# KrishnaswamyLab/MELD

Hardware: AMD Instinct MI355X
Metric: cells/sec through MELD.fit_transform (kNN+Chebyshev) (higher is better)
Workload: dtype f64

## Files before the change

### include/meld_hip.h

```cpp
#ifndef MELD_HIP_H
#define MELD_HIP_H

#include <stddef.h>
#include <stdint.h>

#ifdef __cplusplus
extern "C" {
#endif

#define MELD_OK 0
#define MELD_ERR_INVALID (-1)
#define MELD_ERR_UNSUPPORTED (-2)
#define MELD_ERR_HIP (-3)

typedef void* meld_stream_t;

int meld_abi_version(void);
const char* meld_last_error(void);
int meld_device_count(void);


int meld_knn_padded_dim(int d);
int meld_knn_tile_refs(void);
int meld_knn_block_queries(void);
int meld_knn_row_capacity(int ksel);
double meld_knn_error_coef(int d);

int meld_col_sums_f64(const double* X, int64_t N, int d, double* sums, meld_stream_t stream);
size_t meld_col_stats_temp_bytes(int d);
int meld_col_stats_f64(const double* X, int64_t N, int d, double* sums, double* mins, double* maxs, void* temp, size_t temp_bytes,
                       meld_stream_t stream);

int meld_knn_prepare_refs(const double* X, int64_t N, int d, const double* mean, int KP, float* Rt,
                          float* norm2, float* norm2_max, meld_stream_t stream);
int meld_knn_prepare_queries(const double* X, int64_t N, int d, const double* mean, int KP,
                             int64_t q_begin, int64_t q_count, float* Q, meld_stream_t stream);

int meld_knn_topk(const float* Q, const float* Rt, int64_t n_ref, int KP, int64_t q_count, int ksel,
                  int32_t* cand_idx, float* cand_d2, int32_t* cand_cnt, meld_stream_t stream);

int meld_knn16_kblocks(int d);
int meld_knn16_tile_refs(void);
int meld_knn16_split_dims(int d);
int meld_frame_max_dims(void);
int meld_cov_sample_f64(const double* X, int64_t N, int d, const double* mean, int64_t stride, double* cov, meld_stream_t stream);
int meld_rotate_rows_f64(const double* X, int64_t N, int d, const double* mean, const double* At, double* out, meld_stream_t stream);
int meld_knn16_block_queries(void);
int meld_knn16_row_capacity(int ksel);
double meld_knn16_error_coef(int nprod, int d);
double meld_knn16_error_coef_const(int nprod, int d);
double meld_knn16_error_coef_lin(int nprod);
size_t meld_knn16_tile_bytes(int d);
size_t meld_knn16_query_bytes(int d);
int meld_knn16_prepare(const double* X, int64_t N, int d, const double* mean, int64_t q_begin,
                       int64_t q_count, void* Rt16, void* Q16, float* Qn, float* norm2, float* norm2_max,
                       float* scale_info, meld_stream_t stream);
int meld_knn16_prepare_scaled(const double* X, int64_t N, int d, const double* mean, const double* col_min, const double* col_max,
                              int64_t q_begin, int64_t q_count, void* Rt16, void* Q16, float* Qn, float* norm2, float* norm2_max,
                              float* scale_info, meld_stream_t stream);
int meld_knn16_prepare_fused(const double* X, int64_t N, int d, const double* mean, const double* col_min, const double* col_max,
                             void* Rt16, void* Q16, float* Qn, float* norm2, float* norm2_max, float* scale_info, void* temp,
                             meld_stream_t stream);
size_t meld_knn16_bounds_bytes(int64_t n_ref, int64_t q_count);
size_t meld_knn16_bounds_temp_bytes(int64_t n_ref, int d, int64_t q_count);
int meld_knn16_bounds(const double* X, int64_t N, int d, const double* mean, const float* scale_info,
                      const float* norm2_max, const void* Rt16, int64_t q_begin, int64_t q_count,
                      const float* thr_seed, const float* q_norm2 ,
                      int nprod, void* temp, void* lb2, meld_stream_t stream);
int meld_knn16_tile_spheres(const double* X, int64_t N, int d, const double* mean, const float* scale_info, void* temp,
                            int64_t tile_begin, int64_t tile_count, meld_stream_t stream);
int meld_knn16_sphere_layout(int64_t n_ref, int d, int64_t* rows, int64_t* row_bytes);
int meld_knn16_bounds_from_spheres(const double* X, int64_t N, int d, const double* mean, const float* scale_info,
                      const float* norm2_max, const void* Rt16, int64_t q_begin, int64_t q_count,
                      const float* thr_seed, const float* q_norm2 ,
                      int nprod, void* temp, void* lb2, meld_stream_t stream);
int meld_knn16_prepare_cross(const double* X, int64_t n_refs, int64_t n_total, int d, const double* mean, int64_t q_begin,
                             int64_t q_count, void* Rt16, void* Q16, float* Qn, float* norm2, float* norm2_max,
                             float* scale_info, meld_stream_t stream);
int meld_knn16_prepare_rows(const double* X, int64_t N, int d, const double* mean, const float* scale_info,
                            int64_t q_begin, const int32_t* rows, int64_t n_rows, void* Q16, float* Qn,
                            meld_stream_t stream);
int meld_knn16_research_thresholds(const int32_t* rows, int64_t n_rows, int64_t q_begin, const int32_t* cand_cnt,
                                   const float* cand_d2, int cap, int ksel, const float* norm2, const float* norm2_max,
                                   double err_coef, double err_lin, double err3, const float* scale_info, float* thr,
                                   meld_stream_t stream);
int meld_knn16_seed_thresholds_mfma(const void* Q16, const float* Qn, const void* Rt16, const float* scale_info,
                                    const float* norm2_max, int64_t n_ref, int d, int64_t q_begin, int64_t q_count,
                                    int knn, double radius_factor, int nprod, int side_tiles, float* thr_init,
                                    meld_stream_t stream);
int meld_knn16_topk(const void* Q16, const float* Qn, const void* Rt16, const float* scale_info,
                    int64_t n_ref, int d, int64_t q_count, int ksel, int nprod, int n_slices, const void* lb2,
                    const float* norm2_max, int64_t q_begin, const float* thr_init, int knn, double radius_factor,
                    int32_t* cand_idx, float* cand_d2, int32_t* cand_cnt, float* cand_thr,
                    uint64_t* tiles_done ,
                    const int32_t* block_order ,
                    meld_stream_t stream);
int meld_knn16_block_work(const void* lb2, const float* thr_seed, int64_t n_ref, int d, int64_t q_count, int nprod,
                          const float* norm2_max, const float* scale_info, int32_t* work, meld_stream_t stream);
int meld_knn16_step_lists(const void* lb2, const float* thr_seed, int64_t n_ref, int d, int64_t q_count, int nprod,
// ... 340 lines not shown
```

### meld_amd/_lib.py

```python
from __future__ import annotations

from ._options import is_set, opt

import ctypes as C
import os

_HERE = os.path.dirname(os.path.abspath(__file__))
LIB_NAME = "libmeld_hip.so"
LIB_PATH = os.path.join(_HERE, LIB_NAME)

_i32, _i64, _f64, _sz, _ptr = C.c_int, C.c_int64, C.c_double, C.c_size_t, C.c_void_p

SIGNATURES = {
    "meld_abi_version": (_i32, []),
    "meld_last_error": (C.c_char_p, []),
    "meld_device_count": (_i32, []),
    "meld_knn_padded_dim": (_i32, [_i32]),
    "meld_knn_tile_refs": (_i32, []),
    "meld_knn_block_queries": (_i32, []),
    "meld_knn_row_capacity": (_i32, [_i32]),
    "meld_col_sums_f64": (_i32, [_ptr, _i64, _i32, _ptr, _ptr]),
    "meld_col_stats_temp_bytes": (_sz, [_i32]),
    "meld_col_stats_f64": (_i32, [_ptr, _i64, _i32, _ptr, _ptr, _ptr, _ptr, _sz, _ptr]),
    "meld_knn_prepare_refs": (_i32, [_ptr, _i64, _i32, _ptr, _i32, _ptr, _ptr, _ptr, _ptr]),
# ... 85 lines not shown
    "meld_csr_transpose_keys": (_i32, [_ptr, _ptr, _ptr, _i32, _i64, _ptr, _ptr, _ptr]),
    "meld_csr_rows_to_dense_f64": (_i32, [_ptr, _ptr, _ptr, _i32, _i64, _i64, _i64, _ptr, _i64, _ptr]),
    "meld_csr_bucket_slots": (_i32, []),
    "meld_coo_scatter_rows": (_i32, [_ptr, _ptr, _i64, _i64, _i64, _ptr, _ptr, _ptr, _ptr]),
    "meld_coo_emit_scatter": (_i32, [_i64, _ptr, _ptr, _i32, _i32, _ptr, _ptr, _i32, _ptr, _ptr, _ptr, _i64, _ptr, _ptr, _ptr, _ptr]),
    "meld_coo_emit_scatter_listed": (_i32, [_ptr, _i32, _ptr, _ptr, _i32, _i32, _ptr, _ptr, _i32, _ptr, _ptr, _ptr, _i64, _ptr, _ptr, _ptr, _ptr]),
    "meld_coo_partition_remote": (_i32, [_ptr, _ptr, _i64, _i64, _i32, _i32, _i64, _ptr, _ptr, _ptr]),
    "meld_csr_rows_sort_merge": (_i32, [_ptr, _i64, _ptr, _ptr, _ptr, _ptr, _i32, _f64, _ptr]),
    "meld_csr_compact_rows": (_i32, [_ptr, _i64, _ptr, _ptr, _ptr, _ptr, _ptr]),
    "meld_csr_rows_sort_merge_sums": (_i32, [_ptr, _i64, _ptr, _ptr, _ptr, _ptr, _i32, _f64, _f64, _ptr, _ptr]),
    "meld_csr_compact_rows_anisotropy": (_i32, [_ptr, _i64, _ptr, _ptr, _ptr, _ptr, _ptr, _f64, _ptr, _ptr]),
    "meld_csr_compact_rows_sums": (_i32, [_ptr, _i64, _ptr, _ptr, _ptr, _ptr, _f64, _ptr, _ptr]),
    "meld_csr_row_sums": (_i32, [_ptr, _ptr, _i64, _f64, _ptr, _ptr]),
    "meld_csr_anisotropy": (_i32, [_ptr, _ptr, _ptr, _i64, _ptr, _i64, _f64, _ptr]),
    "meld_csr_anisotropy_degrees": (_i32, [_ptr, _ptr, _ptr, _i64, _ptr, _i64, _f64, _ptr, _ptr]),
    "meld_extend_rows_temp_bytes": (_sz, [_i64, _i64]),
    "meld_extend_rows": (_i32, [_ptr, _ptr, _i64, _i64, _i64, _i64, _ptr, _ptr, _ptr, _ptr, _ptr, _sz, _ptr]),
    "meld_extend_apply": (_i32, [_ptr, _ptr, _ptr, _ptr, _i64, _ptr, _i64, _i32, _ptr, _ptr, _ptr]),
    "meld_spmm_dot_slots": (_i32, []),
    "meld_cheby_step": (_i32, [_ptr, _i32, _ptr, _i64, _ptr, _ptr, _ptr, _f64, _f64, _f64, _f64, _ptr, _ptr]),
    "meld_lanczos_steps": (_i32, [_ptr, _ptr, _ptr, _ptr, _ptr, _ptr, _ptr, _i32, _i32, _ptr, _ptr, _ptr]),
    "meld_lanczos_spmv": (_i32, [_ptr, _ptr, _i64, _ptr, _ptr, _ptr, _ptr, _ptr]),
    "meld_lanczos_alpha": (_i32, [_ptr, _ptr, _ptr, _ptr, _i32, _ptr]),
    "meld_lanczos_axpy": (_i32, [_ptr, _ptr, _i64, _ptr, _ptr, _ptr]),
    "meld_lanczos_beta": (_i32, [_ptr, _ptr, _ptr, _ptr, _i32, _ptr]),
    "meld_lanczos_fold": (_i32, [_ptr, _ptr, _ptr, _ptr, _i32, _ptr]),
    "meld_lanczos_axpy3": (_i32, [_ptr, _ptr, _ptr, _i64, _ptr, _ptr, _ptr]),
    "meld_pt_geometry": (_i32, [_ptr, _ptr, _ptr, _ptr]),
    "meld_pt_num_blocks": (_i32, [_i64]),
    "meld_pt_seg_len": (_i64, [_i32]),
    "meld_pt_stream_len": (_i64, [_i64, _i32]),
    "meld_pt_desc_len": (_i64, [_i32]),
    "meld_pt_build": (_i32, [_ptr, _ptr, _ptr, _i64, _i64, _i64, _i32, _ptr, _ptr, _ptr, _ptr]),
    "meld_cheby_step_wide": (_i32, [_ptr, _i32, _ptr, _i64, _ptr, _ptr, _f64, _f64, _f64, _ptr]),
    "meld_block_max_blocks": (_i32, []),
    "meld_block_gram_f64": (_i32, [_ptr, _i64, _ptr, _i64, _i64, _i32, _ptr, _i32, _ptr, _ptr]),
    "meld_block_rotate_f64": (_i32, [_ptr, _i64, _ptr, _i64, _i32, _ptr, _i64, _ptr]),
    "meld_block_residuals_f64": (_i32, [_ptr, _ptr, _i64, _ptr, _i64, _i32, _ptr, _i32, _ptr, _ptr]),
    "meld_kmeans_max_blocks": (_i32, []),
    "meld_kmeans_assign": (_i32, [_ptr, _i64, _i32, _ptr, _i32, _ptr, _ptr, _ptr, _ptr, _i32, _ptr]),
    "meld_kmeans_wide_max_d": (_i32, []),
    "meld_kmeans_wide_max_k": (_i32, []),
    "meld_kmeans_wide_assign": (_i32, [_ptr, _i64, _i64, _i32, _ptr, _i32, _ptr, _ptr, _ptr, _ptr]),
    "meld_kmeans_wide_sums": (_i32, [_ptr, _i64, _i64, _i32, _ptr, _ptr, _i32, _ptr, _ptr]),
    "meld_scale_f64": (_i32, [_ptr, _f64, _ptr, _i64, _ptr]),
    "meld_axpby_f64": (_i32, [_f64, _ptr, _f64, _ptr, _i64, _ptr, _ptr]),
    "meld_normalize_rows_l1": (_i32, [_ptr, _ptr, _i64, _i32, _ptr]),
    "meld_assign_nearest": (_i32, [_ptr, _i64, _i32, _ptr, _i32, _ptr, _ptr, _ptr, _ptr]),
    "meld_chain_order": (_i32, [_ptr, _i64, _i32, _i32, _ptr, _ptr]),
    "meld_gather_rows_f64": (_i32, [_ptr, _ptr, _i64, _i32, _ptr, _ptr]),
    "meld_frame_max_dims": (_i32, []),
    "meld_cov_sample_f64": (_i32, [_ptr, _i64, _i32, _ptr, _i64, _ptr, _ptr]),
    "meld_rotate_rows_f64": (_i32, [_ptr, _i64, _i32, _ptr, _ptr, _ptr, _ptr]),
    "meld_argsort_u32_temp_bytes": (_sz, [_i64]),
    "meld_argsort_u32": (_i32, [_ptr, _i64, _i32, _ptr, _ptr, _ptr, _sz, _ptr]),
    "meld_order_starts": (_i32, [_ptr, _i64, _i32, _ptr, _ptr]),
    "meld_order_pick_centroids": (_i32, [_ptr, _i64, _i32, _ptr, _ptr, _i32, _i32, _ptr, _ptr]),
    "meld_order_update_keys": (_i32, [_ptr, _ptr, _ptr, _i64, _i32, _ptr]),
    "meld_rccl_available": (_i32, []),
    "meld_rccl_unique_id": (_i32, [_ptr]),
    "meld_rccl_comm_create": (_i32, [_ptr, _i32, _i32, _ptr]),
    "meld_rccl_comm_destroy": (_i32, [_ptr]),
    "meld_rccl_all_gather": (_i32, [_ptr, _ptr, _ptr, _sz, _ptr]),
    "meld_rccl_all_reduce_sum_f64": (_i32, [_ptr, _ptr, _sz, _ptr]),
    "meld_cheby_run": (_i32, [_ptr, _ptr, _i64, _i64, _i32, _ptr, _ptr, _ptr, _ptr, _i32, _f64, _f64, _ptr, _ptr]),
    "meld_lanczos_steps_sharded": (_i32, [_ptr, _ptr, _i64, _i64, _ptr, _ptr, _ptr, _ptr, _ptr, _ptr, _ptr, _i32, _i32, _ptr]),
    "meld_factorize_max_groups": (_i32, []),
    "meld_factorize_max_words": (_i32, []),
    "meld_factorize_temp_bytes": (_sz, [_i64]),
    "meld_factorize_labels": (_i32, [_ptr, _i64, _i32, _ptr, _sz, _ptr, _ptr]),
    "meld_factorize_codes": (_i32, [_ptr, _i64, _ptr, _ptr, _ptr]),
    "meld_indicator_signal": (_i32, [_ptr, _ptr, _ptr, _i64, _i64, _i32, _ptr, _ptr]),
    "meld_scatter_rows_f64": (_i32, [_ptr, _ptr, _i64, _i32, _ptr, _ptr]),
    "meld_cc_round": (_i32, [_ptr, _ptr, _i64, _ptr, _ptr, _ptr]),
    "meld_cc_minima": (_i32, [_ptr, _ptr, _i64, _ptr, _ptr, _ptr, _ptr]),
    "meld_cc_labels": (_i32, [_ptr, _ptr, _ptr, _ptr, _ptr, _i64, _ptr, _ptr, _ptr]),
    "meld_subgraph_count": (_i32, [_ptr, _ptr, _ptr, _i64, _ptr, _ptr]),
    "meld_subgraph_fill": (_i32, [_ptr, _ptr, _ptr, _ptr, _i64, _ptr, _ptr, _ptr, _ptr]),
    "meld_diffuse_max_cols": (_i32, []),
    "meld_diffuse_step": (_i32, [_ptr, _ptr, _ptr, _ptr, _ptr, _i64, _ptr, _i64, _ptr, _i64, _i32, _ptr]),
    "meld_minplus_max_cols": (_i32, []),
    "meld_minplus_step": (_i32, [_ptr, _ptr, _ptr, _i64, _ptr, _i64, _ptr, _i64, _i32, _ptr, _ptr]),
    "meld_edge_lengths_l2": (_i32, [_ptr, _ptr, _i64, _ptr, _i64, _i32, _ptr, _ptr]),
    "meld_landmark_max": (_i32, []),
    "meld_landmark_merge_count": (_i32, [_ptr, _ptr, _i64, _i64, _ptr, _i32, _ptr, _i32, _ptr, _ptr, _ptr]),
    "meld_landmark_merge_fill": (_i32, [_ptr, _ptr, _ptr, _i64, _ptr, _ptr, _ptr, _ptr, _ptr, _ptr]),
    "meld_landmark_gram": (_i32, [_ptr, _ptr, _ptr, _i64, _ptr, _ptr, _ptr, _i32, _ptr, _ptr, _ptr, _ptr]),
    "meld_smacof_max_dim": (_i32, []),
    "meld_smacof_step": (_i32, [_ptr, _i64, _i32, _i32, _ptr, _ptr, _ptr, _ptr]),
    "meld_louvain_lanes": (_i32, [_i64, _i64]),
    "meld_louvain_move_blocks": (_i64, [_i64, _i32]),
    "meld_louvain_move": (_i32, [_ptr, _ptr, _ptr, _i64, _ptr, _ptr, _ptr, _ptr, _f64, _f64, _i32, _i32, _ptr, _ptr, _ptr, _ptr, _ptr, _ptr, _ptr]),
    "meld_louvain_totals": (_i32, [_ptr, _ptr, _i64, _i64, _ptr, _ptr, _ptr, _ptr]),
    "meld_louvain_heads": (_i32, [_ptr, _ptr, _i64, _ptr, _ptr]),
    "meld_louvain_renumber": (_i32, [_ptr, _ptr, _ptr, _ptr, _i64, _ptr, _ptr, _ptr]),
    "meld_louvain_contract_keys": (_i32, [_ptr, _ptr, _i64, _ptr, _ptr, _ptr]),
    "meld_modularity_terms": (_i32, [_ptr, _ptr, _ptr, _i64, _ptr, _ptr, _ptr, _ptr]),
}


class PtLayout(C.Structure):

    _fields_ = [("blk_row", _ptr), ("blk_ntile", _ptr), ("blk_ndist", _ptr), ("seg", _ptr), ("list_cols", _ptr),
                ("pval", _ptr), ("pidx", _ptr), ("nb", C.c_int32), ("pval32", _ptr), ("stream_len", C.c_int64), ("cdesc", _ptr)]


# ... 42 lines not shown
```

### meld_amd/csrc/frame.hip

```cpp
#include "common.hpp"

namespace meld {

constexpr int FR_ROWS = 64;
constexpr int FR_DMAX = 64;

__global__ __launch_bounds__(256) void cov_sample_kernel(const double* __restrict__ X, int64_t n_s, int64_t stride, int d,
                                                         const double* __restrict__ mean, double* __restrict__ out) {
  __shared__ double sx[FR_ROWS][FR_DMAX + 1];
  const int tid = threadIdx.x;
  const int64_t s0 = (int64_t)blockIdx.x * FR_ROWS;
  const int cnt = (int)min((int64_t)FR_ROWS, n_s - s0);
  for (int u = tid; u < FR_ROWS * d; u += 256) {
    const int r = u / d, k = u - r * d;
    sx[r][k] = r < cnt ? X[(s0 + r) * stride * d + k] - mean[k] : 0.0;
  }
  __syncthreads();
  for (int p = tid; p < d * d; p += 256) {
    const int i = p / d, j = p - i * d;
    if (j < i) continue;
    double acc = 0.0;
    for (int r = 0; r < FR_ROWS; ++r) acc = fma(sx[r][i], sx[r][j], acc);
    atomicAdd(out + p, acc);
  }
}

typedef double f64x8 __attribute__((ext_vector_type(8)));
typedef const __attribute__((address_space(4))) f64x8* const_f64x8_ptr;
constexpr int FR_LD = FR_DMAX + 1;
constexpr int FR_NQ = FR_ROWS * FR_DMAX / 256;
constexpr int FR_CPG = FR_DMAX / 4;
__global__ __launch_bounds__(256) void rotate_rows_kernel(const double* __restrict__ X, int64_t N, int d, const double* __restrict__ mean,
                                                          const double* __restrict__ At, double* __restrict__ out, int64_t tiles_per_wg) {
  __shared__ double sx[FR_ROWS][FR_LD];
  const int tid = threadIdx.x, lane = tid & 63;
  const int w = __builtin_amdgcn_readfirstlane(tid >> 6);
  const int cpg = (d + 3) >> 2;
  const int j0 = w * cpg;
  const int k8n = (d + 7) >> 3;
  const double mk = (lane < d) ? mean[lane] : 0.0;
  const int64_t n_tiles = (N + FR_ROWS - 1) / FR_ROWS;
  const int64_t t_begin = (int64_t)blockIdx.x * tiles_per_wg, t_end = min(n_tiles, t_begin + tiles_per_wg);
  double xv[FR_NQ];
  auto fetch = [&](int64_t t) __attribute__((always_inline)) {
    const int64_t row0 = t * FR_ROWS;
#pragma unroll
    for (int q = 0; q < FR_NQ; ++q) {
      const int u = tid + 256 * q, rr = u >> 6, k = u & 63;
      xv[q] = (t < t_end && row0 + rr < N && k < d) ? X[(row0 + rr) * d + k] : mk;
    }
  };
  fetch(t_begin);
  for (int64_t t = t_begin; t < t_end; ++t) {
    const int64_t row0 = t * FR_ROWS;
    const int cnt = (int)min((int64_t)FR_ROWS, N - row0);
    __syncthreads();
#pragma unroll
    for (int q = 0; q < FR_NQ; ++q) {
      const int u = tid + 256 * q, rr = u >> 6, k = u & 63;
      sx[rr][k] = xv[q] - mk;
    }
    fetch(t + 1);
    __syncthreads();
    double xr[FR_DMAX];
#pragma unroll
    for (int k = 0; k < FR_DMAX; ++k) xr[k] = sx[lane][k];
    double res[FR_CPG];
#pragma unroll
    for (int c4 = 0; c4 < FR_CPG; c4 += 4) {
      double acc[4] = {0.0, 0.0, 0.0, 0.0};
      if (c4 < cpg) {
        const_f64x8_ptr arow[4];
#pragma unroll
        for (int i = 0; i < 4; ++i)
          arow[i] = (const_f64x8_ptr)(uintptr_t)(At + (size_t)min(j0 + c4 + i, d - 1) * FR_DMAX);
#pragma unroll
        for (int k8 = 0; k8 < FR_DMAX / 8; ++k8) {
          if (k8 < k8n) {
            f64x8 av[4];
#pragma unroll
            for (int i = 0; i < 4; ++i) av[i] = arow[i][k8];
#pragma unroll
            for (int e = 0; e < 8; ++e)
#pragma unroll
              for (int i = 0; i < 4; ++i) acc[i] = fma(xr[8 * k8 + e], av[i][e], acc[i]);
          }
        }
      }
#pragma unroll
      for (int i = 0; i < 4; ++i) res[c4 + i] = acc[i];
    }
    __syncthreads();
#pragma unroll
    for (int c = 0; c < FR_CPG; ++c)
      if (c < cpg && j0 + c < d) sx[lane][j0 + c] = res[c];
    __syncthreads();
#pragma unroll
    for (int q = 0; q < FR_NQ; ++q) {
      const int u = tid + 256 * q, rr = u >> 6, k = u & 63;
      if (rr < cnt && k < d) out[(row0 + rr) * d + k] = sx[rr][k];
    }
  }
}

}

using namespace meld;

extern "C" int meld_frame_max_dims(void) { return FR_DMAX; }

extern "C" int meld_cov_sample_f64(const double* X, int64_t N, int d, const double* mean, int64_t stride, double* cov, meld_stream_t stream) {
  MELD_CHECK_ARG(X && mean && cov && N > 0 && d > 0 && d <= FR_DMAX && stride >= 1, "meld_cov_sample_f64: bad arguments (d <= %d)", FR_DMAX);
  const int64_t n_s = (N + stride - 1) / stride;
  hipLaunchKernelGGL(cov_sample_kernel, dim3((unsigned)ceil_div(n_s, FR_ROWS)), dim3(256), 0, S(stream), X, n_s, stride, d, mean, cov);
  MELD_LAUNCH_CHECK("cov_sample_kernel");
  return MELD_OK;
}

extern "C" int meld_rotate_rows_f64(const double* X, int64_t N, int d, const double* mean, const double* At, double* out, meld_stream_t stream) {
  MELD_CHECK_ARG(X && mean && At && out && N > 0 && d > 0 && d <= FR_DMAX && X != out, "meld_rotate_rows_f64: bad arguments (d <= %d)", FR_DMAX);
  const int64_t tiles = ceil_div(N, FR_ROWS);
  const int64_t per = ceil_div(tiles, (int64_t)1024);
  hipLaunchKernelGGL(rotate_rows_kernel, dim3((unsigned)ceil_div(tiles, per)), dim3(256), 0, S(stream), X, N, d, mean, At, out, per);
  MELD_LAUNCH_CHECK("rotate_rows_kernel");
  return MELD_OK;
}
```

### meld_amd/graph.py

```python
from __future__ import annotations

from ._options import opt

import math
import time

from types import SimpleNamespace

import numpy as np
import torch

from ._lib import check, get_lib, ptr
from .knn_plan import SearchOptions, bucket_route, plan_knn_search, search_nprod, sphere_layout

__all__ = ["DeviceGraph", "build_knn_graph", "default_ksel", "EVENTS", "record_events"]

EVENTS = {"enabled": False, "pairs": []}


def record_events(enabled=True):
    EVENTS["enabled"] = bool(enabled)
    EVENTS["pairs"] = []


# ... 499 lines not shown
    tmp = torch.empty(tb, dtype=torch.uint8, device=x.device)
    check(lib.meld_exclusive_scan_i32_i64(ptr(x), ptr(out), n, ptr(tmp), tb, st), "meld_exclusive_scan_i32_i64")
    return out


class HipOps:

    name = "hip"

    def __init__(self, device=None, search=None, prune=None, nprod=None, spmm=None):
        self.lib = get_lib()
        self.spmm = spmm
        o = SearchOptions.from_env(search=search, prune=prune, nprod=nprod)
        self.search, self.nprod, self.prune, self.rotate, self.rotate_min_cells = o.search, o.nprod, o.prune, o.rotate, o.rotate_min_cells
        self.radius_cut, self.seed, self.seeded_bounds, self.block_order = o.radius_cut, o.seed, o.seeded_bounds, o.block_order
        if not torch.cuda.is_available():
            raise RuntimeError("meld_amd needs a ROCm GPU (MI355X); there is no CPU fallback")
        self.device = torch.device("cuda", torch.cuda.current_device()) if device is None else torch.device(device)

    def col_stats(self, X):
        N, d = int(X.shape[0]), int(X.shape[1])
        out = torch.empty(3, d, dtype=torch.float64, device=X.device)
        tb = self.lib.meld_col_stats_temp_bytes(d)
        tmp = torch.empty(tb, dtype=torch.uint8, device=X.device)
        check(self.lib.meld_col_stats_f64(ptr(X), N, d, ptr(out[0]), ptr(out[1]), ptr(out[2]), ptr(tmp), tb, _stream()), "meld_col_stats_f64")
        return out[0], out[1], out[2]

    def frame_axes_async(self, X, col_stats):
        lib = self.lib
        N, d = int(X.shape[0]), int(X.shape[1])
        if col_stats is None or d > int(lib.meld_frame_max_dims()) or not plan_knn_search(lib, N, d, 0, N, 1, 2, options=self).frame:
            return None
        st = _stream()
        mean = col_stats[0] / N
        cov = torch.zeros(d, d, dtype=torch.float64, device=X.device)
        check(lib.meld_cov_sample_f64(ptr(X), N, d, ptr(mean), max(1, N // 32768), ptr(cov), st), "meld_cov_sample_f64")
        host = torch.empty(d, d, dtype=torch.float64, pin_memory=True)
        host.copy_(cov, non_blocking=True)
        done = torch.cuda.Event()
        done.record()

        def finish(lead):
            done.synchronize()
            evals, evecs = _eigh_one_thread(host.numpy())
            tot = float(evals.sum())
            if not np.isfinite(tot) or tot <= 0.0 or float(evals[-lead:].sum()) < 0.5 * tot:
                return False
            At = np.zeros((d, int(lib.meld_frame_max_dims())))
            At[:, :d] = evecs[:, ::-1].T
            return torch.from_numpy(At).to(X.device, non_blocking=True)

        return finish

    def principal_frame(self, X, mean, lead, comm=None, axes=None):
        lib, st = self.lib, _stream()
        N, d = int(X.shape[0]), int(X.shape[1])
        if axes is not None and (comm is None or getattr(comm, "world", 1) == 1):
            At = axes(lead)
            if At is False:
                return None
            out = torch.empty_like(X)
            check(lib.meld_rotate_rows_f64(ptr(X), N, d, ptr(mean), ptr(At), ptr(out), st), "meld_rotate_rows_f64")
            return out
        wide = d > int(lib.meld_frame_max_dims())
        stride = max(1, N // 32768)
        if wide:
            Xs = X[::stride] - mean
            cov = torch.triu(Xs.T @ Xs)
            del Xs
        else:
            cov = torch.zeros(d, d, dtype=torch.float64, device=X.device)
            check(lib.meld_cov_sample_f64(ptr(X), N, d, ptr(mean), stride, ptr(cov), st), "meld_cov_sample_f64")
        if comm is not None and getattr(comm, "world", 1) > 1:
            if comm.rank != 0:
                cov.zero_()
            comm.all_reduce_sum(cov)
        evals, evecs = _eigh_one_thread(cov.cpu().numpy())
        tot = float(evals.sum())
        if not np.isfinite(tot) or tot <= 0.0 or float(evals[-lead:].sum()) < 0.5 * tot:
            return None
        if wide:
            V = torch.from_numpy(np.ascontiguousarray(evecs[:, ::-1])).to(X.device)
            return torch.addmm(-(mean @ V), X, V)
        At = np.zeros((d, int(lib.meld_frame_max_dims())))
        At[:, :d] = evecs[:, ::-1].T
        At = torch.from_numpy(At).to(X.device)
        out = torch.empty_like(X)
        check(lib.meld_rotate_rows_f64(ptr(X), N, d, ptr(mean), ptr(At), ptr(out), st), "meld_rotate_rows_f64")
        return out

    def directed_kernel_coo(self, X, q_begin, q_count, knn, decay, thresh, ksel, tm=None, force_fallback=False, n_refs=None, assemble=False, comm=None,
                            bw_scale=1.0, bw_fixed=None, col_stats=None, knn_max=None, symm=(0, 0.0), count_rows_ge=None, frame_axes=None,
                            anisotropy=None):
        N = int(X.shape[0])
        NR = int(n_refs) if n_refs is not None else N
        if n_refs is not None and not (0 < NR <= q_begin and q_begin + q_count <= N):
            raise ValueError("cross search: the queries must lie behind the n_refs references")
        a = SimpleNamespace(X=X, N=N, d=int(X.shape[1]), NR=NR, cross=n_refs is not None, q_begin=q_begin, q_count=q_count, knn=knn, decay=decay,
                            thresh=thresh, bw_scale=bw_scale, bw_fixed=bw_fixed, knn_max=knn_max, force_fallback=force_fallback,
                            col_stats=col_stats, frame_axes=frame_axes, tm=tm or _Timer(False), assemble=bool(assemble), rows_fused=True)
        out = self._directed_kernel(a, ksel, comm, assemble, symm, count_rows_ge, anisotropy)
        if out is None:
            a.rows_fused = False
            out = self._directed_kernel(a, ksel, comm, assemble, symm, count_rows_ge, anisotropy)
            out[3]["fused_rows_recovered"] = True
        return out

    def _directed_kernel(self, a, ksel, comm, assemble, symm, count_rows_ge, anisotropy):
        q_count, force_fallback = a.q_count, a.force_fallback
        r = self._search_and_refine(a, ksel, comm)
        retry_from = None
        if r.n_flag > max(1024, q_count // 100) and ksel < 128 and r.plan.search == "f16x3" and not force_fallback:
            retry_from, ksel = (ksel, r.n_flag), 128
            r = self._search_and_refine(a, ksel, None)
        s = self._exact_sweep(a, r, count_rows_ge)
        keys, vals, assembled = self._emit(a, r, s, ksel, assemble, symm, anisotropy)
        if r.buckets is not None and assembled is None and r.m_main + s.fb_total > 0:
            return None
        p, c = r.plan, r.cands
        info = dict(ksel=int(ksel), KP=int(c.KP), search=p.search, nprod=p.nprod, n_flagged_rows=r.n_flag,
                    fused_rows=p.fused_rows if p.fused_rows != "sort+emit" or getattr(c, "raw", None) is not None else "emit",
                    prune=p.prune, radius_cut=p.radius_cut, seed=p.seed != "none", seeded_bounds=p.seeded_bounds, block_order=p.block_order != "none",
                    step_lists=p.lists != "none", principal_frame=p.frame, two_phase=p.two_pass, n_rows_bandwidth_recomputed=s.n_rebandwidth,
                    n_researched_rows=r.n_flag_stage1 if p.stage2 else 0, nnz_directed=r.m_main + s.fb_total,
                    wave_tiles_done=r.tiles_done_h, blocks_past_partial_test=r.blocks_on_h, pairs_past_filter=r.pairs_kept_h)
        if s.rows_at_least is not None:
            info["rows_with_at_least"] = s.rows_at_least
        if assembled is not None:
            info["assembled"] = assembled
        if retry_from is not None:
            info["ksel_retry_from"], info["n_flagged_rows_first_try"] = int(retry_from[0]), int(retry_from[1])
        return keys, vals, r.bw, info

    def _search_and_refine(self, a, ksel, comm):
        lib, dev = self.lib, a.X.device
        nprod = search_nprod(self.nprod, a.d)
        resident = lib.meld_knn16_resident_blocks(a.d, nprod) if lib.meld_knn16_kblocks(a.d) > 0 and nprod in (1, 3) else 0
        plan = plan_knn_search(lib, a.N, a.d, a.q_begin, a.q_count, a.knn, ksel, options=self, cross=a.cross, bandwidth=a.bw_fixed is not None,
                               world=getattr(comm, "world", 1) if comm is not None else 1, resident=resident,
                               assemble=a.assemble and a.rows_fused, free_bytes=torch.cuda.mem_get_info(dev)[0] if a.assemble and a.rows_fused else 0,
                               x_aligned=a.X.data_ptr() % 16 == 0)
        a.tm.start()
# ... 51 lines not shown
        return SimpleNamespace(plan=plan, idx=cand_idx, d2=cand_d2, cnt=cand_cnt, thr=None, cap=cap, err_coef=1e-6, err_lin=0.0, KP=a.d,
                               norm2=norm2, nmax=nmax, tiles_done=None, research=None)

    def _candidates_f32(self, a, plan, ksel, mean, norm2, nmax):
        lib, st, dev, X, N, d = self.lib, _stream(), a.X.device, a.X, a.N, a.d
        KP = lib.meld_knn_padded_dim(d)
        if KP < 0:
            check(KP, "meld_knn_padded_dim")
        TS, BQ = lib.meld_knn_tile_refs(), lib.meld_knn_block_queries()
        cap = lib.meld_knn_row_capacity(ksel)
        if cap < 0:
            check(cap, "meld_knn_row_capacity")
        n_tiles = (N + TS - 1) // TS
        Rt = torch.empty(n_tiles * KP * TS, dtype=torch.float32, device=dev)
        check(lib.meld_knn_prepare_refs(ptr(X), N, d, ptr(mean), KP, ptr(Rt), ptr(norm2), ptr(nmax), st), "meld_knn_prepare_refs")
        q_pad = ((a.q_count + BQ - 1) // BQ) * BQ
        Q = torch.empty(q_pad * KP, dtype=torch.float32, device=dev)
        check(lib.meld_knn_prepare_queries(ptr(X), N, d, ptr(mean), KP, a.q_begin, a.q_count, ptr(Q), st), "meld_knn_prepare_queries")
        a.tm.stop("prepare")
        cand_idx = torch.empty(q_pad * cap, dtype=torch.int32, device=dev)
        cand_d2 = torch.empty(q_pad * cap, dtype=torch.float32, device=dev)
        cand_cnt = torch.empty(q_pad, dtype=torch.int32, device=dev)
        with _EventSpan("knn_topk", N=N, d=d, q=a.q_count):
            check(lib.meld_knn_topk(ptr(Q), ptr(Rt), N, KP, a.q_count, ksel, ptr(cand_idx), ptr(cand_d2), ptr(cand_cnt), st), "meld_knn_topk")
        return SimpleNamespace(plan=plan, idx=cand_idx, d2=cand_d2, cnt=cand_cnt, thr=None, cap=cap, err_coef=lib.meld_knn_error_coef(d), err_lin=0.0,
                               KP=KP, norm2=norm2, nmax=nmax, tiles_done=None, research=None)

    def _candidates_f16x3(self, a, plan, ksel, comm, mean, col_min, col_max, norm2, nmax):
        lib, dev = self.lib, a.X.device
        cap = lib.meld_knn16_row_capacity(ksel)
        if cap < 0:
            check(cap, "meld_knn16_row_capacity")
        plan, o, nmax = self._operands16(a, plan, comm, mean, col_min, col_max, norm2, nmax)
        c = SimpleNamespace(plan=plan, cap=cap, err_coef=lib.meld_knn16_error_coef_const(plan.nprod, a.d), err_lin=lib.meld_knn16_error_coef_lin(plan.nprod),
                            KP=16 * o.KB, norm2=norm2, nmax=nmax, research=o if plan.stage2 else None)
        c.idx = torch.empty(o.q_pad * cap, dtype=torch.int32, device=dev)
        c.d2 = torch.empty(o.q_pad * cap, dtype=torch.float32, device=dev)
        c.cnt = torch.empty(o.q_pad, dtype=torch.int32, device=dev)
        c.thr, rfac = None, 1.0
        if plan.radius_cut:
            c.thr = torch.full((o.q_pad,), float("inf"), dtype=torch.float32, device=dev)
            rfac = max(_radius_factor(a.decay, a.thresh) * float(a.bw_scale), 1.0)
        c.tiles_done = torch.zeros(4, dtype=torch.int64, device=dev)
        seeds = self._start_thresholds(a, plan, o, c, rfac)
        lists = self._step_lists(a, plan, o, seeds, nmax, comm)
        self._search16(a, plan, o, c, ksel, seeds, rfac, lists)
        return c

    def _operands16(self, a, plan, comm, mean, col_min, col_max, norm2, nmax):
        lib, st, dev, X, N, d = self.lib, _stream(), a.X.device, a.X, a.N, a.d
        KB, TS, BQ = lib.meld_knn16_kblocks(d), lib.meld_knn16_tile_refs(), lib.meld_knn16_block_queries()
        o = SimpleNamespace(X_s=X, mean_s=mean, KB=KB, BQ=BQ, n_tiles=(a.NR + TS - 1) // TS, q_pad=((a.q_count + BQ - 1) // BQ) * BQ)
        if plan.frame:
            X_s = self.principal_frame(X, mean, int(lib.meld_knn16_split_dims(d)), comm, axes=a.frame_axes)
            if X_s is None:
                plan = plan.without_frame()
            else:
                sums_s, col_min, col_max = self.col_stats(X_s)
                o.X_s, o.mean_s = X_s, sums_s / N
        o.Rt = torch.empty(o.n_tiles * lib.meld_knn16_tile_bytes(d), dtype=torch.uint8, device=dev)
        o.Q = torch.empty(o.q_pad * lib.meld_knn16_query_bytes(d), dtype=torch.uint8, device=dev)
        o.Qn = torch.empty(o.q_pad, dtype=torch.float32, device=dev)
        o.scale_info = torch.empty(4, dtype=torch.float32, device=dev)
        tail = (a.q_begin, a.q_count, ptr(o.Rt), ptr(o.Q), ptr(o.Qn), ptr(norm2), ptr(nmax), ptr(o.scale_info), st)
        if a.cross:
            check(lib.meld_knn16_prepare_cross(ptr(X), a.NR, N, d, ptr(mean), *tail), "meld_knn16_prepare_cross")
        elif plan.fused_operands:
            o.spheres = torch.empty(lib.meld_knn16_bounds_temp_bytes(N, d, a.q_count), dtype=torch.uint8, device=dev)
            check(lib.meld_knn16_prepare_fused(ptr(o.X_s), N, d, ptr(o.mean_s), ptr(col_min), ptr(col_max), ptr(o.Rt), ptr(o.Q), ptr(o.Qn), ptr(norm2),
                                               ptr(nmax), ptr(o.scale_info), ptr(o.spheres), st), "meld_knn16_prepare_fused")
        elif col_min is not None:
            check(lib.meld_knn16_prepare_scaled(ptr(o.X_s), N, d, ptr(o.mean_s), ptr(col_min), ptr(col_max), *tail), "meld_knn16_prepare_scaled")
        else:
            check(lib.meld_knn16_prepare(ptr(o.X_s), N, d, ptr(o.mean_s), *tail), "meld_knn16_prepare")
        a.tm.stop("prepare")
        return plan, o, nmax

    def _start_thresholds(self, a, plan, o, c, rfac):
        lib, st, dev = self.lib, _stream(), a.X.device
        if plan.seed == "bandwidth":
            rad = (a.bw_fixed[a.q_begin : a.q_begin + a.q_count] * float(a.bw_scale)).clamp_(min=float(np.finfo(float).eps)) * _radius_factor(a.decay, a.thresh)
            nmx = c.nmax.to(torch.float64)
            e_row = float(c.err_coef) * nmx + float(c.err_lin) * torch.sqrt(c.norm2[a.q_begin : a.q_begin + a.q_count].to(torch.float64) * nmx)
            seeds = torch.full((o.q_pad,), float("inf"), dtype=torch.float32, device=dev)
            seeds[: a.q_count] = ((rad * rad + 1.01 * e_row) * o.scale_info[0].to(torch.float64) ** 2 * (1.0 + 1e-5)).to(torch.float32)
            if o.q_pad > a.q_count:
                seeds[a.q_count :] = seeds[a.q_count - 1]
            return seeds
        if plan.seed == "mfma":
            seeds = torch.empty(o.q_pad, dtype=torch.float32, device=dev)
            check(lib.meld_knn16_seed_thresholds_mfma(ptr(o.Q), ptr(o.Qn), ptr(o.Rt), ptr(o.scale_info), ptr(c.nmax), a.N, a.d, a.q_begin, a.q_count, a.knn,
                                                      rfac, plan.nprod, 0, ptr(seeds), st), "meld_knn16_seed_thresholds_mfma")
            a.tm.stop("seed")
            return seeds
        return None

    def _step_lists(self, a, plan, o, seeds, nmax, comm):
        if not plan.prune:
            return None, None, None, None
        lib, st, dev, N, d = self.lib, _stream(), a.X.device, a.N, a.d
        X_s, mean_s, n_tiles, n_blocks = o.X_s, o.mean_s, o.n_tiles, o.q_pad // o.BQ
        spheres_ready = getattr(o, "spheres", None) is not None
        tmpb = o.spheres if spheres_ready else torch.empty(lib.meld_knn16_bounds_temp_bytes(N, d, a.q_count), dtype=torch.uint8, device=dev)
        if plan.bounds == "bounds_from_spheres":
            rows_c, row_b = sphere_layout(lib, N, d)
            per = rows_c // comm.world
            t0s = min(comm.rank * per, n_tiles)
            t1s = min(t0s + per, n_tiles)
            tmpb.zero_()
            check(lib.meld_knn16_tile_spheres(ptr(X_s), N, d, ptr(mean_s), ptr(o.scale_info), ptr(tmpb), t0s, max(t1s - t0s, 0), st), "meld_knn16_tile_spheres")
            parts = (tmpb[: rows_c * row_b], tmpb[rows_c * row_b : rows_c * (row_b + 4)], tmpb[rows_c * (row_b + 4) : rows_c * (row_b + 8)])
            for arr, width in zip(parts, (row_b, 4, 4)):
# ... 792 lines not shown
```

Before: 29.20 million.

## Rotate rows with f64 MFMA and fuse column stats into the frame rotation

Replaces the LDS-based rotate_rows kernel with an MFMA f64 16x16x4 kernel that projects centred rows onto the principal axes. The same pass also computes per-column sum, min and max, followed by a small combine kernel. This removes the separate col_stats pass over the rotated matrix. It adds a temp buffer, a second launch and some duplicated allocations per call, and because the accumulation order changes, results may differ in the last bits.

```diff
diff --git a/include/meld_hip.h b/include/meld_hip.h
--- a/include/meld_hip.h
+++ b/include/meld_hip.h
@@ -45,6 +45,9 @@
 int meld_frame_max_dims(void);
 int meld_cov_sample_f64(const double* X, int64_t N, int d, const double* mean, int64_t stride, double* cov, meld_stream_t stream);
 int meld_rotate_rows_f64(const double* X, int64_t N, int d, const double* mean, const double* At, double* out, meld_stream_t stream);
+size_t meld_frame_rotate_temp_bytes(int d);
+int meld_frame_rotate_stats_f64(const double* X, int64_t N, int d, const double* mean, const double* At, double* out, double* col_sum,
+                                double* col_min, double* col_max, double* mean_out, void* temp, size_t temp_bytes, meld_stream_t stream);
 int meld_knn16_block_queries(void);
 int meld_knn16_row_capacity(int ksel);
 double meld_knn16_error_coef(int nprod, int d);
diff --git a/meld_amd/_lib.py b/meld_amd/_lib.py
--- a/meld_amd/_lib.py
+++ b/meld_amd/_lib.py
@@ -161,6 +161,8 @@
     "meld_frame_max_dims": (_i32, []),
     "meld_cov_sample_f64": (_i32, [_ptr, _i64, _i32, _ptr, _i64, _ptr, _ptr]),
     "meld_rotate_rows_f64": (_i32, [_ptr, _i64, _i32, _ptr, _ptr, _ptr, _ptr]),
+    "meld_frame_rotate_temp_bytes": (_sz, [_i32]),
+    "meld_frame_rotate_stats_f64": (_i32, [_ptr, _i64, _i32, _ptr, _ptr, _ptr, _ptr, _ptr, _ptr, _ptr, _ptr, _sz, _ptr]),
     "meld_argsort_u32_temp_bytes": (_sz, [_i64]),
     "meld_argsort_u32": (_i32, [_ptr, _i64, _i32, _ptr, _ptr, _ptr, _sz, _ptr]),
     "meld_order_starts": (_i32, [_ptr, _i64, _i32, _ptr, _ptr]),
diff --git a/meld_amd/csrc/frame.hip b/meld_amd/csrc/frame.hip
--- a/meld_amd/csrc/frame.hip
+++ b/meld_amd/csrc/frame.hip
@@ -25,82 +25,134 @@
   }
 }
 
-typedef double f64x8 __attribute__((ext_vector_type(8)));
-typedef const __attribute__((address_space(4))) f64x8* const_f64x8_ptr;
-constexpr int FR_LD = FR_DMAX + 1;
-constexpr int FR_NQ = FR_ROWS * FR_DMAX / 256;
-constexpr int FR_CPG = FR_DMAX / 4;
-__global__ __launch_bounds__(256) void rotate_rows_kernel(const double* __restrict__ X, int64_t N, int d, const double* __restrict__ mean,
-                                                          const double* __restrict__ At, double* __restrict__ out, int64_t tiles_per_wg) {
-  __shared__ double sx[FR_ROWS][FR_LD];
-  const int tid = threadIdx.x, lane = tid & 63;
-  const int w = __builtin_amdgcn_readfirstlane(tid >> 6);
-  const int cpg = (d + 3) >> 2;
-  const int j0 = w * cpg;
-  const int k8n = (d + 7) >> 3;
-  const double mk = (lane < d) ? mean[lane] : 0.0;
-  const int64_t n_tiles = (N + FR_ROWS - 1) / FR_ROWS;
-  const int64_t t_begin = (int64_t)blockIdx.x * tiles_per_wg, t_end = min(n_tiles, t_begin + tiles_per_wg);
-  double xv[FR_NQ];
-  auto fetch = [&](int64_t t) __attribute__((always_inline)) {
-    const int64_t row0 = t * FR_ROWS;
-#pragma unroll
-    for (int q = 0; q < FR_NQ; ++q) {
-      const int u = tid + 256 * q, rr = u >> 6, k = u & 63;
-      xv[q] = (t < t_end && row0 + rr < N && k < d) ? X[(row0 + rr) * d + k] : mk;
-    }
-  };
-  fetch(t_begin);
-  for (int64_t t = t_begin; t < t_end; ++t) {
-    const int64_t row0 = t * FR_ROWS;
-    const int cnt = (int)min((int64_t)FR_ROWS, N - row0);
-    __syncthreads();
-#pragma unroll
-    for (int q = 0; q < FR_NQ; ++q) {
-      const int u = tid + 256 * q, rr = u >> 6, k = u & 63;
-      sx[rr][k] = xv[q] - mk;
-    }
-    fetch(t + 1);
-    __syncthreads();
-    double xr[FR_DMAX];
-#pragma unroll
-    for (int k = 0; k < FR_DMAX; ++k) xr[k] = sx[lane][k];
-    double res[FR_CPG];
-#pragma unroll
-    for (int c4 = 0; c4 < FR_CPG; c4 += 4) {
-      double acc[4] = {0.0, 0.0, 0.0, 0.0};
-      if (c4 < cpg) {
-        const_f64x8_ptr arow[4];
-#pragma unroll
-        for (int i = 0; i < 4; ++i)
-          arow[i] = (const_f64x8_ptr)(uintptr_t)(At + (size_t)min(j0 + c4 + i, d - 1) * FR_DMAX);
-#pragma unroll
-        for (int k8 = 0; k8 < FR_DMAX / 8; ++k8) {
-          if (k8 < k8n) {
-            f64x8 av[4];
-#pragma unroll
-            for (int i = 0; i < 4; ++i) av[i] = arow[i][k8];
-#pragma unroll
-            for (int e = 0; e < 8; ++e)
-#pragma unroll
-              for (int i = 0; i < 4; ++i) acc[i] = fma(xr[8 * k8 + e], av[i][e], acc[i]);
+typedef double double4_t __attribute__((ext_vector_type(4)));
+constexpr int FR_THREADS = 256;
+constexpr int FR_WAVES = FR_THREADS / 64;
+constexpr int FR_GROUP = 16;
+constexpr int FR_MAX_BLOCKS = 2048;
+constexpr int FR_V_LD = 80;
+
+template <int T, bool STATS>
+__global__ __launch_bounds__(FR_THREADS) void frame_rotate_kernel(const double* __restrict__ X, int64_t N, int d, const double* __restrict__ mean,
+                                                                  const double* __restrict__ At, double* __restrict__ out, int64_t per,
+                                                                  double* __restrict__ part) {
+  __shared__ double s_v[16 * T * FR_V_LD];
+  const int lane = threadIdx.x & 63, wv = threadIdx.x >> 6;
+  const int c = lane & 15, g = lane >> 4;
+  for (int e = threadIdx.x; e < 16 * T * FR_DMAX; e += FR_THREADS) {
+    const int j = e / FR_DMAX, k = e % FR_DMAX;
+    if (k < 16 * T) s_v[k * FR_V_LD + j] = (j < d && k < d) ? At[j * FR_DMAX + k] : 0.0;
+  }
+  double mk[4 * T];
+#pragma unroll
+  for (int s = 0; s < 4 * T; ++s) mk[s] = 4 * s + g < d ? mean[4 * s + g] : 0.0;
+  __syncthreads();
+  const int ks = (d + 3) >> 2;
+  const int64_t r_begin = (int64_t)blockIdx.x * per, r_end = min(N, r_begin + per);
+  double lsum[T], lmin[T], lmax[T];
+#pragma unroll
+  for (int tj = 0; tj < T; ++tj) lsum[tj] = 0.0, lmin[tj] = INFINITY, lmax[tj] = -INFINITY;
+  for (int64_t i0 = r_begin + (int64_t)wv * FR_GROUP; i0 < r_end; i0 += FR_WAVES * FR_GROUP) {
+    const double* xr = X + min(i0 + c, r_end - 1) * d;
+    double a[4 * T];
+#pragma unroll
+    for (int s = 0; s < 4 * T; ++s) a[s] = xr[min(4 * s + g, d - 1)];
+#pragma unroll
+    for (int s = 0; s < 4 * T; ++s) a[s] = (i0 + c < r_end && 4 * s + g < d) ? a[s] - mk[s] : 0.0;
+    double4_t acc[T];
+#pragma unroll
+    for (int tj = 0; tj < T; ++tj) acc[tj] = double4_t{0.0, 0.0, 0.0, 0.0};
+    auto step = [&](int s) __attribute__((always_inline)) {
+#pragma unroll
+      for (int tj = 0; tj < T; ++tj)
+        acc[tj] = __builtin_amdgcn_mfma_f64_16x16x4f64(a[s], s_v[(4 * s + g) * FR_V_LD + 16 * tj + c], acc[tj], 0, 0, 0);
+    };
+#pragma unroll
+    for (int b = 0; b < T; ++b) {
+      if (ks >= 4 * b + 4) {
+#pragma unroll
+        for (int u = 0; u < 4; ++u) step(4 * b + u);
+      } else {
+#pragma unroll
+        for (int u = 0; u < 4; ++u)
+          if (4 * b + u < ks) step(4 * b + u);
+      }
+    }
+#pragma unroll
+    for (int tj = 0; tj < T; ++tj)
+#pragma unroll
+      for (int q = 0; q < 4; ++q) {
+        const int64_t row = i0 + g + 4 * q;
+        if (row < r_end && 16 * tj + c < d) {
+          const double v = acc[tj][q];
+          out[row * d + 16 * tj + c] = v;
+          if constexpr (STATS) {
+            lsum[tj] += v;
+            lmin[tj] = fmin(lmin[tj], v);
+            lmax[tj] = fmax(lmax[tj], v);
           }
         }
       }
-#pragma unroll
-      for (int i = 0; i < 4; ++i) res[c4 + i] = acc[i];
-    }
+  }
+  if constexpr (STATS) {
     __syncthreads();
 #pragma unroll
-    for (int c = 0; c < FR_CPG; ++c)
-      if (c < cpg && j0 + c < d) sx[lane][j0 + c] = res[c];
+    for (int tj = 0; tj < T; ++tj) {
+      double* p = s_v + ((wv * 4 + g) * 16 * T + 16 * tj + c) * 3;
+      p[0] = lsum[tj], p[1] = lmin[tj], p[2] = lmax[tj];
+    }
     __syncthreads();
-#pragma unroll
-    for (int q = 0; q < FR_NQ; ++q) {
-      const int u = tid + 256 * q, rr = u >> 6, k = u & 63;
-      if (rr < cnt && k < d) out[(row0 + rr) * d + k] = sx[rr][k];
-    }
-  }
+    const int j = threadIdx.x;
+    if (j < d) {
+      double ts = 0.0, tmn = INFINITY, tmx = -INFINITY;
+      for (int u = 0; u < FR_WAVES * 4; ++u) {
+        const double* p = s_v + (u * 16 * T + j) * 3;
+        ts += p[0];
+        tmn = fmin(tmn, p[1]);
+        tmx = fmax(tmx, p[2]);
+      }
+      const size_t nb = gridDim.x;
+      part[(0 * nb + blockIdx.x) * d + j] = ts;
+      part[(1 * nb + blockIdx.x) * d + j] = tmn;
+      part[(2 * nb + blockIdx.x) * d + j] = tmx;
+    }
+  }
+}
+
+__global__ __launch_bounds__(FR_THREADS) void frame_stats_combine_kernel(const double* __restrict__ part, int n_blocks, int d, int64_t N,
+                                                                         double* __restrict__ sums, double* __restrict__ mins,
+                                                                         double* __restrict__ maxs, double* __restrict__ mean_out) {
+  __shared__ double ps[FR_THREADS], pmin[FR_THREADS], pmax[FR_THREADS];
+  const int c = blockIdx.x, tid = threadIdx.x;
+  const int run = (n_blocks + FR_THREADS - 1) / FR_THREADS;
+  double ts = 0.0, tmn = INFINITY, tmx = -INFINITY;
+  for (int b = tid * run; b < min(n_blocks, (tid + 1) * run); ++b) {
+    ts += part[((size_t)0 * n_blocks + b) * d + c];
+    tmn = fmin(tmn, part[((size_t)1 * n_blocks + b) * d + c]);
+    tmx = fmax(tmx, part[((size_t)2 * n_blocks + b) * d + c]);
+  }
+  ps[tid] = ts, pmin[tid] = tmn, pmax[tid] = tmx;
+  __syncthreads();
+  for (int w = 1; w < FR_THREADS; w <<= 1) {
+    if ((tid & (2 * w - 1)) == 0) {
+      ps[tid] += ps[tid + w];
+      pmin[tid] = fmin(pmin[tid], pmin[tid + w]);
+      pmax[tid] = fmax(pmax[tid], pmax[tid + w]);
+    }
+    __syncthreads();
+  }
+  if (tid == 0) {
+    sums[c] = ps[0];
+    mins[c] = pmin[0];
+    maxs[c] = pmax[0];
+    mean_out[c] = ps[0] / (double)N;
+  }
+}
+
+static inline int64_t frame_rows_per_block(int64_t N) {
+  const int64_t groups = ceil_div(N, (int64_t)(FR_WAVES * FR_GROUP));
+  const int64_t blocks = groups < FR_MAX_BLOCKS ? groups : FR_MAX_BLOCKS;
+  return ceil_div(ceil_div(N, blocks), (int64_t)FR_GROUP) * FR_GROUP;
 }
 
 }
@@ -117,11 +169,40 @@
   return MELD_OK;
 }
 
+extern "C" size_t meld_frame_rotate_temp_bytes(int d) { return sizeof(double) * 3 * (size_t)FR_MAX_BLOCKS * (size_t)(d > 0 ? d : 1); }
+
+extern "C" int meld_frame_rotate_stats_f64(const double* X, int64_t N, int d, const double* mean, const double* At, double* out, double* col_sum,
+                                           double* col_min, double* col_max, double* mean_out, void* temp, size_t temp_bytes,
+                                           meld_stream_t stream) {
+  MELD_CHECK_ARG(X && mean && At && out && N > 0 && d > 0 && d <= FR_DMAX && X != out, "meld_frame_rotate_stats_f64: bad arguments (d <= %d)",
+                 FR_DMAX);
+  const bool stats = col_sum || col_min || col_max || mean_out;
+  MELD_CHECK_ARG(!stats || (col_sum && col_min && col_max && mean_out && temp && temp_bytes >= meld_frame_rotate_temp_bytes(d)),
+                 "meld_frame_rotate_stats_f64: the four statistics go together, with temp of meld_frame_rotate_temp_bytes(d) bytes");
+  const int64_t per = frame_rows_per_block(N);
+  const unsigned grid = (unsigned)ceil_div(N, per);
+  double* part = reinterpret_cast<double*>(temp);
+  const int T = d <= 16 ? 1 : d <= 32 ? 2 : 4;
+#define MELD_FRAME_CASE(TT)                                                                                                                \
+  if (T == TT) {                                                                                                                           \
+    if (stats)                                                                                                                             \
+      hipLaunchKernelGGL((frame_rotate_kernel<TT, true>), dim3(grid), dim3(FR_THREADS), 0, S(stream), X, N, d, mean, At, out, per, part);  \
+    else                                                                                                                                   \
+      hipLaunchKernelGGL((frame_rotate_kernel<TT, false>), dim3(grid), dim3(FR_THREADS), 0, S(stream), X, N, d, mean, At, out, per, part); \
+  }
+  MELD_FRAME_CASE(1)
+  MELD_FRAME_CASE(2)
+  MELD_FRAME_CASE(4)
+#undef MELD_FRAME_CASE
+  MELD_LAUNCH_CHECK("frame_rotate_kernel");
+  if (stats) {
+    hipLaunchKernelGGL(frame_stats_combine_kernel, dim3((unsigned)d), dim3(FR_THREADS), 0, S(stream), part, (int)grid, d, N, col_sum, col_min,
+                       col_max, mean_out);
+    MELD_LAUNCH_CHECK("frame_stats_combine_kernel");
+  }
+  return MELD_OK;
+}
+
 extern "C" int meld_rotate_rows_f64(const double* X, int64_t N, int d, const double* mean, const double* At, double* out, meld_stream_t stream) {
-  MELD_CHECK_ARG(X && mean && At && out && N > 0 && d > 0 && d <= FR_DMAX && X != out, "meld_rotate_rows_f64: bad arguments (d <= %d)", FR_DMAX);
-  const int64_t tiles = ceil_div(N, FR_ROWS);
-  const int64_t per = ceil_div(tiles, (int64_t)1024);
-  hipLaunchKernelGGL(rotate_rows_kernel, dim3((unsigned)ceil_div(tiles, per)), dim3(256), 0, S(stream), X, N, d, mean, At, out, per);
-  MELD_LAUNCH_CHECK("rotate_rows_kernel");
-  return MELD_OK;
-}
+  return meld_frame_rotate_stats_f64(X, N, d, mean, At, out, nullptr, nullptr, nullptr, nullptr, nullptr, 0, stream);
+}
diff --git a/meld_amd/graph.py b/meld_amd/graph.py
--- a/meld_amd/graph.py
+++ b/meld_amd/graph.py
@@ -575,6 +575,17 @@
 
         return finish
 
+    def _rotate_with_stats(self, X, mean, At):
+        lib = self.lib
+        N, d = int(X.shape[0]), int(X.shape[1])
+        out = torch.empty_like(X)
+        stats = torch.empty(4, d, dtype=torch.float64, device=X.device)
+        tb = lib.meld_frame_rotate_temp_bytes(d)
+        tmp = torch.empty(tb, dtype=torch.uint8, device=X.device)
+        check(lib.meld_frame_rotate_stats_f64(ptr(X), N, d, ptr(mean), ptr(At), ptr(out), ptr(stats[0]), ptr(stats[1]), ptr(stats[2]), ptr(stats[3]),
+                                              ptr(tmp), tb, _stream()), "meld_frame_rotate_stats_f64")
+        return out, (stats[0], stats[1], stats[2], stats[3])
+
     def principal_frame(self, X, mean, lead, comm=None, axes=None):
         lib, st = self.lib, _stream()
         N, d = int(X.shape[0]), int(X.shape[1])
@@ -582,9 +593,7 @@
             At = axes(lead)
             if At is False:
                 return None
-            out = torch.empty_like(X)
-            check(lib.meld_rotate_rows_f64(ptr(X), N, d, ptr(mean), ptr(At), ptr(out), st), "meld_rotate_rows_f64")
-            return out
+            return self._rotate_with_stats(X, mean, At)
         wide = d > int(lib.meld_frame_max_dims())
         stride = max(1, N // 32768)
         if wide:
@@ -604,13 +613,12 @@
             return None
         if wide:
             V = torch.from_numpy(np.ascontiguousarray(evecs[:, ::-1])).to(X.device)
-            return torch.addmm(-(mean @ V), X, V)
+            out = torch.addmm(-(mean @ V), X, V)
+            sums, col_min, col_max = self.col_stats(out)
+            return out, (sums, col_min, col_max, sums / N)
         At = np.zeros((d, int(lib.meld_frame_max_dims())))
         At[:, :d] = evecs[:, ::-1].T
-        At = torch.from_numpy(At).to(X.device)
-        out = torch.empty_like(X)
-        check(lib.meld_rotate_rows_f64(ptr(X), N, d, ptr(mean), ptr(At), ptr(out), st), "meld_rotate_rows_f64")
-        return out
+        return self._rotate_with_stats(X, mean, torch.from_numpy(At).to(X.device))
 
     def directed_kernel_coo(self, X, q_begin, q_count, knn, decay, thresh, ksel, tm=None, force_fallback=False, n_refs=None, assemble=False, comm=None,
                             bw_scale=1.0, bw_fixed=None, col_stats=None, knn_max=None, symm=(0, 0.0), count_rows_ge=None, frame_axes=None,
@@ -768,12 +776,11 @@
         KB, TS, BQ = lib.meld_knn16_kblocks(d), lib.meld_knn16_tile_refs(), lib.meld_knn16_block_queries()
         o = SimpleNamespace(X_s=X, mean_s=mean, KB=KB, BQ=BQ, n_tiles=(a.NR + TS - 1) // TS, q_pad=((a.q_count + BQ - 1) // BQ) * BQ)
         if plan.frame:
-            X_s = self.principal_frame(X, mean, int(lib.meld_knn16_split_dims(d)), comm, axes=a.frame_axes)
-            if X_s is None:
+            framed = self.principal_frame(X, mean, int(lib.meld_knn16_split_dims(d)), comm, axes=a.frame_axes)
+            if framed is None:
                 plan = plan.without_frame()
             else:
-                sums_s, col_min, col_max = self.col_stats(X_s)
-                o.X_s, o.mean_s = X_s, sums_s / N
+                o.X_s, (_, col_min, col_max, o.mean_s) = framed
         o.Rt = torch.empty(o.n_tiles * lib.meld_knn16_tile_bytes(d), dtype=torch.uint8, device=dev)
         o.Q = torch.empty(o.q_pad * lib.meld_knn16_query_bytes(d), dtype=torch.uint8, device=dev)
         o.Qn = torch.empty(o.q_pad, dtype=torch.float32, device=dev)
```

New measurement: 29.78 million (median of 4 runs). 2.0% higher.
